# KirillHit/snn_for_object_detection

Hardware: AMD Instinct MI355X
Metric: event-frames/sec (BxT) SODa-3M GEN1 304x240 fwd+bwd (higher is better)
Workload: dtype f32 (16-bit split products)

## Files before the change

### snn_for_object_detection_amd/csrc/conv_halo.hip

```cpp
#include <stdlib.h>
#include <type_traits>
#include "conv_common.h"

namespace {

constexpr int HBM_ = 128;
constexpr int HCELLS = 288;
constexpr int HPIECE = HCELLS * 64;
constexpr int NPASS = HCELLS / 32;
static_assert(NPASS == 9, "one halo staging pass per tap");

struct HaloGeom {
    int64_t ldx, ldy, ld_add, ld_add2;
    int N, H, W, Cin, Cout;
    int PW, PH;
    int G;
    int group_cells;
    int tiles_per_group, tiles, tiles_per_xcd, ntiles_n;
    unsigned magic_pw, magic_ph;
    int out_vec;
    double* bn_partial;
    int OH, OW;
    int tiles_x, tiles_img;
    float x_th;
};

__device__ __forceinline__ unsigned udiv_small(unsigned n, unsigned magic) { return __umulhi(n, magic); }

template <bool F16>
__device__ __forceinline__ void split4(const f32x4& v, u32x2& hi, u32x2& lo) {
#pragma unroll
    for (int e = 0; e < 4; e += 2) {
        if constexpr (F16) {
            const float a = v[e] * kF16ActScale, b = v[e + 1] * kF16ActScale;
            const f16x2 ph = __builtin_convertvector(f32x2{a, b}, f16x2);
            const f16x2 pl = __builtin_convertvector(f32x2{a - (float)ph[0], b - (float)ph[1]}, f16x2);
            hi[e >> 1] = __builtin_bit_cast(unsigned, ph);
            lo[e >> 1] = __builtin_bit_cast(unsigned, pl);
        } else {
            f32x2 rest = {v[e], v[e + 1]};
            const bf16x2 ph = __builtin_convertvector(rest, bf16x2);
            const unsigned bits = __builtin_bit_cast(unsigned, ph);
            rest[0] -= __builtin_bit_cast(float, bits << 16);
            rest[1] -= __builtin_bit_cast(float, bits & 0xffff0000u);
            const bf16x2 pl = __builtin_convertvector(rest, bf16x2);
            hi[e >> 1] = bits;
            lo[e >> 1] = __builtin_bit_cast(unsigned, pl);
        }
    }
}

__device__ __forceinline__ double partner8(double v) {
    const u32x2 u = __builtin_bit_cast(u32x2, v);
    const u32x2 o = {(unsigned)__builtin_amdgcn_update_dpp(0, (int)u[0], 0x128, 0xf, 0xf, false),
                     (unsigned)__builtin_amdgcn_update_dpp(0, (int)u[1], 0x128, 0xf, 0xf, false)};
    return __builtin_bit_cast(double, o);
}
__device__ __forceinline__ double partner16(double v) {
    const u32x2 u = __builtin_bit_cast(u32x2, v);
    const u32x2 o = {__builtin_amdgcn_permlane16_swap(u[0], u[0], false, false)[0],
                     __builtin_amdgcn_permlane16_swap(u[1], u[1], false, false)[0]};
    return __builtin_bit_cast(double, o);
}
__device__ __forceinline__ double partner32(double v) {
    const u32x2 u = __builtin_bit_cast(u32x2, v);
    const u32x2 o = {__builtin_amdgcn_permlane32_swap(u[0], u[0], false, false)[0],
                     __builtin_amdgcn_permlane32_swap(u[1], u[1], false, false)[0]};
    return __builtin_bit_cast(double, o);
}

__device__ __forceinline__ int cell_slot_off(int cell, int slot) { return cell * 64 + ((slot ^ ((cell >> 2) & 3)) << 4); }


constexpr int RTH = 4, RTW = 32, RPITCH = RTW + 2, RCELLS = (RTH + 2) * RPITCH;

template <int CO, bool F16, int ABL = 0, bool RECT = false, bool SBF = false, bool XSP = false>
__global__ __launch_bounds__(kThreads, 2) void k_conv_halo3(const float* __restrict__ x,
                                                           const unsigned char* __restrict__ wimg,
                                                           float* __restrict__ y, HaloGeom g,
                                                           const float* __restrict__ addend,
                                                           const float* __restrict__ addend2) {
    constexpr int WM = CO == 32 ? 4 : 2, WN = 4 / WM, TM = CO == 32 ? 1 : 2, TN = CO == 32 ? 1 : CO / 64;
    static_assert(CO == 32 || CO == 64 || CO == 128, "channel tile");
    constexpr int BTILE = (CO / 32) * 4096;
    constexpr int NDMA = (CO / 32) * 4 / 4;
    constexpr int ES = SBF ? 2 : 4;
    static_assert(!SBF || (!F16 && ABL == 0), "bf16 storage: bf16 MFMA, plain variant");
    static_assert(!XSP || (F16 && !SBF && ABL == 0), "spikes from potentials: the forward arithmetic, plain variant");
    constexpr int HC = RECT ? (RCELLS + 31) / 32 * 32 : HCELLS;
    constexpr int HP = HC * 64;
    constexpr int RED_BYTES = (F16 || SBF) ? 4 * (CO == 128 ? 64 : 32) * 16 : 0;
    __shared__ __attribute__((aligned(16))) unsigned char smem[2 * HP + 2 * BTILE + RED_BYTES];
    unsigned char* Aimg = smem;
    unsigned char* Bimg = smem + 2 * HP;

    const int tid = threadIdx.x, lane = tid & 63;
    const int wave = __builtin_amdgcn_readfirstlane(tid >> 6);
    const int wm = wave / WN, wn = wave % WN;
    const int r = lane & 31, h = lane >> 5;

    const int bq = blockIdx.x >> 3;
    const int tile = (blockIdx.x & 7) * g.tiles_per_xcd + bq / g.ntiles_n;
    if (tile >= g.tiles) return;
    const int n0c = (bq % g.ntiles_n) * CO;
    int grp, kt, c0 = 0, x0 = 0, y0 = 0, n0, nb;
    [[maybe_unused]] int ty = 0, tx = 0;
    if constexpr (RECT) {
        n0 = tile / g.tiles_img;
        const int rem = tile - n0 * g.tiles_img;
        ty = rem / g.tiles_x;
        tx = rem - ty * g.tiles_x;
        grp = n0 / g.G;
        kt = (n0 - grp * g.G) * g.tiles_img + rem;
        nb = n0;
    } else {
        grp = tile / g.tiles_per_group;
        kt = tile - grp * g.tiles_per_group;
        c0 = kt * HBM_;
        const int R0g = c0 / g.PW;
        x0 = c0 - R0g * g.PW;
        const int ng = R0g / g.PH;
        y0 = R0g - ng * g.PH;
        n0 = grp * g.G + ng;
        nb = n0 > 0 ? n0 - 1 : 0;
    }
    const int pitch = RECT ? RPITCH : g.PW;

    const int quad = tid & 7;
    const int64_t ipix = (int64_t)g.H * g.W;
    const int64_t xbytes = ((((int64_t)g.N - nb) * ipix - 1) * g.ldx + g.Cin) * ES;
    __amdgpu_buffer_rsrc_t rs_x = __builtin_amdgcn_make_buffer_rsrc(
        reinterpret_cast<char*>(const_cast<float*>(x)) + (int64_t)nb * ipix * g.ldx * ES, 0,
        xbytes > 0x7fffffffLL ? 0x7fffffff : (int)xbytes, 0x00020000);
    unsigned voff[NPASS];
    int awr[NPASS];
#pragma unroll
    for (int p = 0; p < NPASS; ++p) {
        const int cell = p * 32 + (tid >> 3);
        int xx, yy, n;
        bool ok;
        if constexpr (RECT) {
            const int rr = cell / RPITCH, cc = cell - rr * RPITCH;
            yy = ty * RTH - 1 + rr;
            xx = tx * RTW - 1 + cc;
            n = n0;
            ok = cell < RCELLS && yy >= 0 && yy < g.H && xx >= 0 && xx < g.W;
        } else {
            const unsigned u = (unsigned)(x0 + cell + g.PW - 1);
            const unsigned dR = udiv_small(u, g.magic_pw);
            xx = (int)(u - dR * g.PW);
            const unsigned v = (unsigned)(y0 + (int)dR + g.PH - 2);
            const unsigned dn = udiv_small(v, g.magic_ph);
            yy = (int)(v - dn * g.PH);
            n = n0 - 1 + (int)dn;
            ok = n >= 0 && n < g.N && xx < g.W && yy < g.H;
        }
        const int64_t pix = (int64_t)(n - nb) * ipix + (int64_t)yy * g.W + xx;
        voff[p] = ok ? (unsigned)((pix * g.ldx + quad * 4) * ES) : 0x80000000u;
        awr[p] = cell_slot_off(cell, quad >> 1) + (quad & 1) * 8;
    }

    int cellbase[TM];
#pragma unroll
    for (int i = 0; i < TM; ++i)
        cellbase[i] = RECT ? (wm * TM + i + 1) * RPITCH + 1 + r : g.PW + 1 + (wm * TM + i) * 32 + r;
    const int nchunks = g.Cin >> 5;
    const int co_tiles = g.Cout >> 5;
    const unsigned char* wsrc = wimg + (int64_t)(n0c >> 5) * 4096 + lane * 16;
    const unsigned lds_b = (unsigned)(size_t)(__attribute__((address_space(3))) unsigned char*)Bimg;
    auto dma_b = [&](int kk, int buf) {
        if constexpr (SBF)
            if (wave & 1) return;
        const int chunk = kk / 9, tap = kk - chunk * 9;
        const unsigned char* src = wsrc + ((int64_t)(tap * nchunks + chunk) * co_tiles) * 4096 + wave * 1024;
        const unsigned dst = lds_b + buf * BTILE + wave * 1024;
#pragma unroll
        for (int q = 0; q < NDMA; ++q) {
            unsigned keep;
            asm volatile("s_mov_b32 %0, m0\n\ts_mov_b32 m0, %2\n\ts_nop 0\n\tglobal_load_lds_dwordx4 %1, off\n\ts_mov_b32 m0, %0"
                         : "=&s"(keep)
                         : "v"(src + q * 4096), "s"(__builtin_amdgcn_readfirstlane(dst + q * 4096))
                         : "memory");
        }
    };

    using PReg = typename std::conditional<SBF, u32x2, f32x4>::type;
    PReg pf[NPASS];
    auto store_halo = [&]() {
#pragma unroll
        for (int p = 0; p < NPASS; ++p) {
            if constexpr (RECT)
                if (p * 32 >= HC) continue;
            if constexpr (SBF) {
                *reinterpret_cast<u32x2*>(Aimg + awr[p]) = pf[p];
            } else if constexpr (XSP) {
                const u32x2 hi = {(pf[p][0] > g.x_th ? 0x4C00u : 0u) | (pf[p][1] > g.x_th ? 0x4C000000u : 0u),
                                  (pf[p][2] > g.x_th ? 0x4C00u : 0u) | (pf[p][3] > g.x_th ? 0x4C000000u : 0u)};
                *reinterpret_cast<u32x2*>(Aimg + awr[p]) = hi;
            } else {
                u32x2 hi, lo;
                split4<F16>(pf[p], hi, lo);
                *reinterpret_cast<u32x2*>(Aimg + awr[p]) = hi;
                *reinterpret_cast<u32x2*>(Aimg + HP + awr[p]) = lo;
            }
        }
    };
    auto load_pass = [&](int off) -> PReg {
        if constexpr (SBF) return __builtin_bit_cast(u32x2, __builtin_amdgcn_raw_buffer_load_b64(rs_x, off, 0, 0));
        else return __builtin_bit_cast(f32x4, __builtin_amdgcn_raw_buffer_load_b128(rs_x, off, 0, 0));
    };

    f32x16 acc[TM][TN];
#pragma unroll
    for (int i = 0; i < TM; ++i)
#pragma unroll
        for (int j = 0; j < TN; ++j)
#pragma unroll
            for (int e = 0; e < 16; ++e) acc[i][j][e] = 0.f;

    auto kstep = [&](int tapoff, const unsigned char* Bb) {
#pragma unroll
        for (int ks = 0; ks < 2; ++ks) {
            bf16x8 ah[TM], al[TM], bh[TN], bl[TN];
#pragma unroll
            for (int i = 0; i < TM; ++i) {
                const int off = cell_slot_off(cellbase[i] + tapoff, 2 * ks + h);
                if constexpr (ABL & 16) {
                    if (i == 0 && ks == 0) ah[0] = *reinterpret_cast<const bf16x8*>(Aimg + off);
                    ah[i] = ah[0];
                    al[i] = ah[0];
                    continue;
                }
                ah[i] = *reinterpret_cast<const bf16x8*>(Aimg + off);
                if constexpr (!SBF && !XSP) al[i] = *reinterpret_cast<const bf16x8*>(Aimg + HP + off);
            }
#pragma unroll
            for (int j = 0; j < TN; ++j) {
                const int off = (wn * TN + j) * 4096 + ks * 2048 + lane * 16;
                bh[j] = *reinterpret_cast<const bf16x8*>(Bb + off);
                if constexpr (!SBF) bl[j] = *reinterpret_cast<const bf16x8*>(Bb + off + 1024);
            }
#pragma unroll
            for (int i = 0; i < TM; ++i)
#pragma unroll
                for (int j = 0; j < TN; ++j) {
                    if constexpr (SBF) {
                        acc[i][j] = __builtin_amdgcn_mfma_f32_32x32x16_bf16(ah[i], bh[j], acc[i][j], 0, 0, 0);
                    } else if constexpr (XSP) {
                        const f16x8 xah = __builtin_bit_cast(f16x8, ah[i]);
                        const f16x8 xbh = __builtin_bit_cast(f16x8, bh[j]), xbl = __builtin_bit_cast(f16x8, bl[j]);
                        acc[i][j] = __builtin_amdgcn_mfma_f32_32x32x16_f16(xah, xbl, acc[i][j], 0, 0, 0);
                        acc[i][j] = __builtin_amdgcn_mfma_f32_32x32x16_f16(xah, xbh, acc[i][j], 0, 0, 0);
                    } else if constexpr (F16) {
                        const f16x8 xah = __builtin_bit_cast(f16x8, ah[i]), xal = __builtin_bit_cast(f16x8, al[i]);
                        const f16x8 xbh = __builtin_bit_cast(f16x8, bh[j]), xbl = __builtin_bit_cast(f16x8, bl[j]);
                        acc[i][j] = __builtin_amdgcn_mfma_f32_32x32x16_f16(xal, xbh, acc[i][j], 0, 0, 0);
                        acc[i][j] = __builtin_amdgcn_mfma_f32_32x32x16_f16(xah, xbl, acc[i][j], 0, 0, 0);
                        acc[i][j] = __builtin_amdgcn_mfma_f32_32x32x16_f16(xah, xbh, acc[i][j], 0, 0, 0);
                    } else {
                        acc[i][j] = __builtin_amdgcn_mfma_f32_32x32x16_bf16(al[i], bh[j], acc[i][j], 0, 0, 0);
                        acc[i][j] = __builtin_amdgcn_mfma_f32_32x32x16_bf16(ah[i], bl[j], acc[i][j], 0, 0, 0);
                        acc[i][j] = __builtin_amdgcn_mfma_f32_32x32x16_bf16(ah[i], bh[j], acc[i][j], 0, 0, 0);
                    }
                }
        }
    };

    dma_b(0, 0);
#pragma unroll
    for (int p = 0; p < NPASS; ++p) pf[p] = load_pass((int)voff[p]);
    store_halo();
    asm volatile("s_waitcnt vmcnt(0) lgkmcnt(0)\n\ts_barrier" ::: "memory");

    const int nk = nchunks * 9;
#pragma unroll 1
    for (int chunk = 0; chunk < nchunks; ++chunk) {
        const bool more = chunk + 1 < nchunks;
        const int cbytes = (chunk + 1) * 32 * ES;
#pragma unroll
        for (int tap = 0; tap < 9; ++tap) {
            const int kk = chunk * 9 + tap;
            const int cur = kk & 1;
            if constexpr (!(ABL & 1))
                if (kk + 1 < nk) dma_b(kk + 1, cur ^ 1);
            __builtin_amdgcn_sched_barrier(0);
            if constexpr (!(ABL & 4)) {
                if (more) pf[tap] = load_pass((int)(voff[tap] + (unsigned)cbytes));
            }
            __builtin_amdgcn_sched_barrier(0);
            const int kh = tap / 3, kw = tap - 3 * kh;
            kstep((kh - 1) * pitch + (kw - 1), Bimg + cur * BTILE);
            if constexpr (ABL & 2) asm volatile("" ::: "memory");
            else if constexpr (ABL & 4) asm volatile("s_waitcnt vmcnt(0) lgkmcnt(0)\n\ts_barrier" ::: "memory");
            else asm volatile("s_waitcnt vmcnt(0) lgkmcnt(0)\n\ts_barrier" ::: "memory");
        }
        if (more) {
            store_halo();
            asm volatile("s_waitcnt lgkmcnt(0)\n\ts_barrier" ::: "memory");
        }
    }

    constexpr int EW = TN * 32 + 4;
    constexpr int LPR = TN * 8;
    constexpr int RPP = 64 / LPR;
    float* stage = reinterpret_cast<float*>(smem) + wave * 32 * EW;
    const bool ovec = g.out_vec != 0;
    const int lrow = lane / LPR, c4 = (lane % LPR) * 4;
    const int nch = n0c + wn * TN * 32 + c4;
    const int cells_left = g.group_cells - c0;
    double ssum[4] = {0.0, 0.0, 0.0, 0.0}, qsum[4] = {0.0, 0.0, 0.0, 0.0};
    const bool stats = (F16 || SBF) && g.bn_partial != nullptr;
    auto cell_pixel = [&](int m, int64_t& pix) -> bool {
        int xx, yy, n;
        bool ok;
        if constexpr (RECT) {
            yy = ty * RTH + (m >> 5);
            xx = tx * RTW + (m & 31);
            n = n0;
            ok = yy < g.H && xx < g.W && nch < g.Cout;
        } else {
            const unsigned u = (unsigned)(x0 + m);
            const unsigned dR = udiv_small(u, g.magic_pw);
            xx = (int)(u - dR * g.PW);
            const unsigned v = (unsigned)(y0 + (int)dR);
            const unsigned dn = udiv_small(v, g.magic_ph);
            yy = (int)(v - dn * g.PH);
            n = n0 + (int)dn;
            ok = m < cells_left && xx < g.W && yy < g.H && n < g.N && nch < g.Cout;
        }
        pix = ((int64_t)n * g.H + yy) * g.W + xx;
        return ok;
    };
    typedef SnnStore<SBF> St;
    constexpr int NPS = 32 / RPP;
    const bool prefetch_add = ovec && (addend != nullptr || addend2 != nullptr) && !(ABL & 8);
#pragma unroll
    for (int i = 0; i < TM; ++i) {
        f32x4 pa1[NPS], pa2[NPS];
        int64_t ppix[NPS];
        unsigned okmask = 0;
        if (prefetch_add) {
#pragma unroll
            for (int pass = 0; pass < NPS; ++pass) {
                const bool ok = cell_pixel((wm * TM + i) * 32 + pass * RPP + lrow, ppix[pass]);
                okmask |= ok ? 1u << pass : 0u;
                const int64_t pc = ok ? ppix[pass] : 0;
                const int nc = ok ? nch : 0;
                const f32x4 zero = {0.f, 0.f, 0.f, 0.f};
                pa1[pass] = addend ? St::ld4_last(addend, pc * g.ld_add + nc) : zero;
                pa2[pass] = addend2 ? St::ld4_last(addend2, pc * g.ld_add2 + nc) : zero;
            }
        }
#pragma unroll
        for (int j = 0; j < TN; ++j)
#pragma unroll
            for (int e = 0; e < 16; ++e)
                stage[((e & 3) + 8 * (e >> 2) + 4 * h) * EW + j * 32 + r] = F16 ? acc[i][j][e] * kF16Unscale : acc[i][j][e];
        asm volatile("s_waitcnt lgkmcnt(0)" ::: "memory");
        if (prefetch_add) {
#pragma unroll
            for (int pass = 0; pass < NPS; ++pass) {
                f32x4 val = *reinterpret_cast<const f32x4*>(&stage[(pass * RPP + lrow) * EW + c4]);
                if (addend) val += pa1[pass];
                if (addend2) val += pa2[pass];
                if ((okmask >> pass) & 1u) St::st4(y, ppix[pass] * g.ldy + nch, val);
            }
            asm volatile("s_waitcnt lgkmcnt(0)" ::: "memory");
            continue;
        }
#pragma unroll
        for (int pass = 0; pass < NPS; ++pass) {
            const int row = pass * RPP + lrow;
            int64_t pix;
            const bool ok = cell_pixel((wm * TM + i) * 32 + row, pix);
            f32x4 val = *reinterpret_cast<const f32x4*>(&stage[row * EW + c4]);
            if (!ok) continue;
            if constexpr (ABL & 8) {
                asm volatile("" :: "v"(val[0]), "v"(val[1]), "v"(val[2]), "v"(val[3]));
                continue;
            }
            if (ovec) {
                if (addend) val += St::ld4_last(addend, pix * g.ld_add + nch);
                if (addend2) val += St::ld4_last(addend2, pix * g.ld_add2 + nch);
                St::st4(y, pix * g.ldy + nch, val);
            } else {
#pragma unroll
                for (int q = 0; q < 4; ++q) {
                    float o = val[q];
                    if (addend) o += St::ld1(addend, pix * g.ld_add + nch + q);
                    if (addend2) o += St::ld1(addend2, pix * g.ld_add2 + nch + q);
                    St::st1(y, pix * g.ldy + nch + q, o);
                }
            }
            if (stats) {
#pragma unroll
                for (int q = 0; q < 4; ++q) {
                    const double d = (double)val[q];
                    ssum[q] += d;
                    qsum[q] = fma(d, d, qsum[q]);
                }
            }
        }
        asm volatile("s_waitcnt lgkmcnt(0)" ::: "memory");
    }
    if (stats) {
#pragma unroll
        for (int q = 0; q < 4; ++q) {
            if constexpr (LPR <= 8) {
                ssum[q] += partner8(ssum[q]);
                qsum[q] += partner8(qsum[q]);
            }
            ssum[q] += partner16(ssum[q]);
            qsum[q] += partner16(qsum[q]);
            ssum[q] += partner32(ssum[q]);
            qsum[q] += partner32(qsum[q]);
        }
        double* red = reinterpret_cast<double*>(smem + 2 * HP + 2 * BTILE);
        if (lane >= 48 && lane < 48 + LPR) {
#pragma unroll
            for (int q = 0; q < 4; ++q) {
                red[((wave * LPR + lane - 48) * 4 + q) * 2 + 0] = ssum[q];
                red[((wave * LPR + lane - 48) * 4 + q) * 2 + 1] = qsum[q];
            }
        }
        __syncthreads();
        if (tid < CO) {
            const int wn_ = tid / (TN * 32), cc = tid % (TN * 32);
            double s = 0.0, q2 = 0.0;
#pragma unroll
            for (int wm_ = 0; wm_ < WM; ++wm_) {
                const double* src = red + (((wm_ * WN + wn_) * LPR * 4) + cc) * 2;
                s += src[0];
                q2 += src[1];
            }
            if (n0c + tid < g.Cout) {
                double* dstp = g.bn_partial + snn_bn_partial_index(grp, kt, n0c + tid, g.tiles_per_group, g.Cout);
                dstp[0] = s;
                dstp[1] = q2;
            }
        }
    }
}

constexpr int SPITCH = RTW + 1, SCELLS = (RTH + 1) * SPITCH;
template <bool SBF = false, bool RECT = false>
__global__ __launch_bounds__(kThreads, 2) void k_conv_s2dgrad3(const float* __restrict__ x,
                                                              const unsigned char* __restrict__ wimg,
                                                              float* __restrict__ y,
                                                              HaloGeom g, const float* __restrict__ addend,
                                                              const float* __restrict__ addend2) {
    constexpr int CO = 64, TN = 2;
    constexpr int ES = SBF ? 2 : 4;
    constexpr int BTILE = (CO / 32) * 4096;
    constexpr int NDMA = (CO / 32) * 4 / 4;
    __shared__ __attribute__((aligned(16))) unsigned char smem[2 * HPIECE + 2 * BTILE];
    unsigned char* Aimg = smem;
    unsigned char* Bimg = smem + 2 * HPIECE;

    const int tid = threadIdx.x, lane = tid & 63;
    const int wave = __builtin_amdgcn_readfirstlane(tid >> 6);
    const int r = lane & 31, h = lane >> 5;

    const int bq = blockIdx.x >> 3;
    const int tile = (blockIdx.x & 7) * g.tiles_per_xcd + bq / g.ntiles_n;
    if (tile >= g.tiles) return;
    const int n0c = (bq % g.ntiles_n) * CO;
    int c0 = 0, x0 = 0, y0 = 0, n0;
    [[maybe_unused]] int ty = 0, tx = 0;
    if constexpr (RECT) {
        n0 = tile / g.tiles_img;
        const int rem = tile - n0 * g.tiles_img;
        ty = rem / g.tiles_x;
        tx = rem - ty * g.tiles_x;
    } else {
        c0 = tile * HBM_;
        const int R0g = c0 / g.PW;
        x0 = c0 - R0g * g.PW;
        n0 = R0g / g.PH;
        y0 = R0g - n0 * g.PH;
    }
    const int nb = n0;
    const int pitch = RECT ? SPITCH : g.PW;

    const int quad = tid & 7;
    const int64_t ipix = (int64_t)g.H * g.W;
    const int64_t xbytes = ((((int64_t)g.N - nb) * ipix - 1) * g.ldx + g.Cin) * ES;
    __amdgpu_buffer_rsrc_t rs_x = __builtin_amdgcn_make_buffer_rsrc(
        reinterpret_cast<char*>(const_cast<float*>(x)) + (int64_t)nb * ipix * g.ldx * ES, 0,
        xbytes > 0x7fffffffLL ? 0x7fffffff : (int)xbytes, 0x00020000);
    unsigned voff[NPASS];
    int awr[NPASS];
#pragma unroll
    for (int p = 0; p < NPASS; ++p) {
        const int cell = p * 32 + (tid >> 3);
        int xx, yy, n;
        bool ok;
        if constexpr (RECT) {
            const int rr = cell / SPITCH, cc = cell - rr * SPITCH;
            yy = ty * RTH + rr;
            xx = tx * RTW + cc;
            n = n0;
            ok = cell < SCELLS && xx < g.W && yy < g.H;
        } else {
            const unsigned u = (unsigned)(x0 + cell);
            const unsigned dR = udiv_small(u, g.magic_pw);
            xx = (int)(u - dR * g.PW);
            const unsigned v = (unsigned)(y0 + (int)dR);
            const unsigned dn = udiv_small(v, g.magic_ph);
            yy = (int)(v - dn * g.PH);
            n = n0 + (int)dn;
            ok = n < g.N && xx < g.W && yy < g.H;
        }
        const int64_t pix = (int64_t)(n - nb) * ipix + (int64_t)yy * g.W + xx;
        voff[p] = ok ? (unsigned)((pix * g.ldx + quad * 4) * ES) : 0x80000000u;
        awr[p] = cell_slot_off(cell, quad >> 1) + (quad & 1) * 8;
    }
    const int cellbase = RECT ? wave * SPITCH + r : wave * 32 + r;
    const int nchunks = g.Cin >> 5;
    const int co_tiles = g.Cout >> 5;
    const unsigned char* wsrc = wimg + (int64_t)(n0c >> 5) * 4096 + lane * 16;
    const unsigned lds_b = (unsigned)(size_t)(__attribute__((address_space(3))) unsigned char*)Bimg;
    auto dma_b = [&](int kk, int buf) {
        if constexpr (SBF)
            if (wave & 1) return;
        const int chunk = kk / 9, tap = kk - chunk * 9;
        const unsigned char* src = wsrc + ((int64_t)((8 - tap) * nchunks + chunk) * co_tiles) * 4096 + wave * 1024;
        const unsigned dst = lds_b + buf * BTILE + wave * 1024;
#pragma unroll
        for (int q = 0; q < NDMA; ++q) {
            unsigned keep;
            asm volatile("s_mov_b32 %0, m0\n\ts_mov_b32 m0, %2\n\ts_nop 0\n\tglobal_load_lds_dwordx4 %1, off\n\ts_mov_b32 m0, %0"
                         : "=&s"(keep)
                         : "v"(src + q * 4096), "s"(__builtin_amdgcn_readfirstlane(dst + q * 4096))
                         : "memory");
        }
    };
    using PReg = typename std::conditional<SBF, u32x2, f32x4>::type;
    PReg pf[NPASS];
    auto store_halo = [&]() {
#pragma unroll
        for (int p = 0; p < NPASS; ++p) {
            if constexpr (SBF) {
                *reinterpret_cast<u32x2*>(Aimg + awr[p]) = pf[p];
            } else {
                u32x2 hi, lo;
                split4<false>(pf[p], hi, lo);
                *reinterpret_cast<u32x2*>(Aimg + awr[p]) = hi;
                *reinterpret_cast<u32x2*>(Aimg + HPIECE + awr[p]) = lo;
            }
        }
    };
    auto load_pass = [&](int off) -> PReg {
        if constexpr (SBF) return __builtin_bit_cast(u32x2, __builtin_amdgcn_raw_buffer_load_b64(rs_x, off, 0, 0));
        else return __builtin_bit_cast(f32x4, __builtin_amdgcn_raw_buffer_load_b128(rs_x, off, 0, 0));
    };
    f32x16 acc[4][TN];
#pragma unroll
    for (int c = 0; c < 4; ++c)
#pragma unroll
        for (int j = 0; j < TN; ++j)
#pragma unroll
            for (int e = 0; e < 16; ++e) acc[c][j][e] = 0.f;

    auto kstep = [&](int tapoff, const unsigned char* Bb, f32x16 (&a)[TN]) {
#pragma unroll
        for (int ks = 0; ks < 2; ++ks) {
            const int off = cell_slot_off(cellbase + tapoff, 2 * ks + h);
            const bf16x8 ah = *reinterpret_cast<const bf16x8*>(Aimg + off);
            bf16x8 al = ah;
            if constexpr (!SBF) al = *reinterpret_cast<const bf16x8*>(Aimg + HPIECE + off);
#pragma unroll
            for (int j = 0; j < TN; ++j) {
                const int boff = j * 4096 + ks * 2048 + lane * 16;
                const bf16x8 bh = *reinterpret_cast<const bf16x8*>(Bb + boff);
                if constexpr (!SBF) {
                    const bf16x8 bl = *reinterpret_cast<const bf16x8*>(Bb + boff + 1024);
                    a[j] = __builtin_amdgcn_mfma_f32_32x32x16_bf16(al, bh, a[j], 0, 0, 0);
                    a[j] = __builtin_amdgcn_mfma_f32_32x32x16_bf16(ah, bl, a[j], 0, 0, 0);
                }
                a[j] = __builtin_amdgcn_mfma_f32_32x32x16_bf16(ah, bh, a[j], 0, 0, 0);
            }
        }
    };

    dma_b(0, 0);
#pragma unroll
    for (int p = 0; p < NPASS; ++p) pf[p] = load_pass((int)voff[p]);
    store_halo();
    asm volatile("s_waitcnt vmcnt(0) lgkmcnt(0)\n\ts_barrier" ::: "memory");

    const int nk = nchunks * 9;
#pragma unroll 1
    for (int chunk = 0; chunk < nchunks; ++chunk) {
        const bool more = chunk + 1 < nchunks;
        const int cbytes = (chunk + 1) * 32 * ES;
#pragma unroll
        for (int tap = 0; tap < 9; ++tap) {
            const int kk = chunk * 9 + tap;
            const int cur = kk & 1;
            if (kk + 1 < nk) dma_b(kk + 1, cur ^ 1);
            __builtin_amdgcn_sched_barrier(0);
            if (more) pf[tap] = load_pass((int)(voff[tap] + (unsigned)cbytes));
            __builtin_amdgcn_sched_barrier(0);
            const int kh = tap / 3, kw = tap - 3 * kh;
            const int ph = kh == 1 ? 0 : 1, pw = kw == 1 ? 0 : 1;
            const int dh = kh == 0 ? 1 : 0, dw = kw == 0 ? 1 : 0;
            kstep(dh * pitch + dw, Bimg + cur * BTILE, acc[2 * ph + pw]);
            asm volatile("s_waitcnt vmcnt(0) lgkmcnt(0)\n\ts_barrier" ::: "memory");
        }
        if (more) {
            store_halo();
            asm volatile("s_waitcnt lgkmcnt(0)\n\ts_barrier" ::: "memory");
        }
    }

    constexpr int EW = TN * 32 + 4, LPR = TN * 8, RPP = 64 / LPR;
    float* stage = reinterpret_cast<float*>(smem) + wave * 32 * EW;
    const bool ovec = g.out_vec != 0;
    const int lrow = lane / LPR, c4 = (lane % LPR) * 4;
    const int nch = n0c + c4;
    const int cells_left = g.group_cells - c0;
#pragma unroll
    for (int cls = 0; cls < 4; ++cls) {
        const int ph = cls >> 1, pw = cls & 1;
#pragma unroll
        for (int j = 0; j < TN; ++j)
#pragma unroll
            for (int e = 0; e < 16; ++e)
                stage[((e & 3) + 8 * (e >> 2) + 4 * h) * EW + j * 32 + r] = acc[cls][j][e];
        asm volatile("s_waitcnt lgkmcnt(0)" ::: "memory");
#pragma unroll
        for (int pass = 0; pass < 32 / RPP; ++pass) {
            const int row = pass * RPP + lrow;
            const int m = wave * 32 + row;
            int aa, bb, n;
            bool inside;
            if constexpr (RECT) {
                aa = ty * RTH + wave;
                bb = tx * RTW + row;
                n = n0;
                inside = true;
            } else {
                const unsigned u = (unsigned)(x0 + m);
                const unsigned dR = udiv_small(u, g.magic_pw);
                bb = (int)(u - dR * g.PW);
                const unsigned v = (unsigned)(y0 + (int)dR);
                const unsigned dn = udiv_small(v, g.magic_ph);
                aa = (int)(v - dn * g.PH);
                n = n0 + (int)dn;
                inside = m < cells_left && n < g.N;
            }
            const int hi = 2 * aa + ph, wi = 2 * bb + pw;
            const bool ok = inside && bb < g.W && aa < g.H && hi < g.OH && wi < g.OW && nch < g.Cout;
            f32x4 val = *reinterpret_cast<const f32x4*>(&stage[row * EW + c4]);
            if (!ok) continue;
            const int64_t pix = ((int64_t)n * g.OH + hi) * g.OW + wi;
            typedef SnnStore<SBF> St;
            if (ovec) {
                if (addend) val += St::ld4_last(addend, pix * g.ld_add + nch);
                if (addend2) val += St::ld4_last(addend2, pix * g.ld_add2 + nch);
                St::st4(y, pix * g.ldy + nch, val);
            } else {
#pragma unroll
                for (int q = 0; q < 4; ++q) {
                    float o = val[q];
                    if (addend) o += St::ld1(addend, pix * g.ld_add + nch + q);
                    if (addend2) o += St::ld1(addend2, pix * g.ld_add2 + nch + q);
                    St::st1(y, pix * g.ldy + nch + q, o);
                }
            }
        }
        asm volatile("s_waitcnt lgkmcnt(0)" ::: "memory");
    }
}

template <bool F16>
__global__ void k_weight_frag_image(const float* __restrict__ flat_src, unsigned char* __restrict__ flat_dst,
                                    const int64_t* __restrict__ table, int flip) {
    const int64_t* row = table + (int64_t)blockIdx.y * 4;
    const float* src = flat_src + row[0];
    unsigned char* dst = flat_dst + row[1];
    const int O = (int)row[2], I = (int)row[3];
    const int ot_n = O >> 5, ic_n = I >> 5;
    const int64_t total = (int64_t)9 * ic_n * ot_n * 2 * 64;
    for (int64_t idx = (int64_t)blockIdx.x * blockDim.x + threadIdx.x; idx < total; idx += (int64_t)gridDim.x * blockDim.x) {
        const int lane = (int)(idx & 63);
        const int ks = (int)((idx >> 6) & 1);
        int64_t rest = idx >> 7;
        const int ot = (int)(rest % ot_n); rest /= ot_n;
        const int ic = (int)(rest % ic_n);
        const int tap = (int)(rest / ic_n);
        const int r = lane & 31, h = lane >> 5;
        const int st = flip ? 8 - tap : tap;
        const float* p = src + ((int64_t)(ot * 32 + r) * 9 + st) * I + ic * 32 + ks * 16 + h * 8;
        const f32x4 v0 = *reinterpret_cast<const f32x4*>(p), v1 = *reinterpret_cast<const f32x4*>(p + 4);
        u32x4 hi, lo;
#pragma unroll
// ... 55 lines not shown
static void plan_grid(HaloPlan& p) {
    if (p.tiles * (int64_t)p.ntiles_n + 8 >= 0x7fffffffLL) {
        p.mode = 0;
        return;
    }
    p.tiles_per_xcd = (int)snn_ceil_div(p.tiles, 8);
    const int64_t grid = (int64_t)p.tiles_per_xcd * 8 * p.ntiles_n;
    if (grid > 0x7fffffffLL) p.mode = 0;
    p.grid = (int)grid;
}
static HaloPlan halo_plan(int64_t N, int H, int W, int Cin, int Cout, int G) {
    HaloPlan p = {};
    p.mode = halo_mode(N, H, W, Cin, Cout);
    if (p.mode == 0 || G <= 0 || N % G != 0) return HaloPlan{};
    p.G = G;
    p.co_tile = Cout % 128 == 0 ? 128 : (Cout % 64 == 0 ? 64 : 32);
    p.ntiles_n = Cout / p.co_tile;
    p.tiles_x = (int)snn_ceil_div(W, RTW);
    p.tiles_img = p.tiles_x * (int)snn_ceil_div(H, RTH);
    int64_t tiles;
    if (p.mode == 2) {
        p.tiles_per_group = G * p.tiles_img;
        tiles = N * (int64_t)p.tiles_img;
    } else {
        const int64_t group_cells = (int64_t)G * (H + 1) * (W + 1);
        p.group_cells = (int)group_cells;
        p.tiles_per_group = (int)snn_ceil_div(group_cells, HBM_);
        tiles = (N / G) * p.tiles_per_group;
    }
    if (tiles >= 0x7fffffffLL) return HaloPlan{};
    p.tiles = (int)tiles;
    plan_grid(p);
    return p;
}
static HaloPlan s2dgrad_plan(int64_t N, int H, int W, int Cin, int Ho, int Wo, int Cout) {
    HaloPlan p = {};
    if (!s2dgrad_shape_ok(N, H, W, Cin, Ho, Wo, Cout)) return p;
    p.mode = s2dgrad_rect(Wo) ? 2 : 1;
    p.G = (int)N;
    p.co_tile = 64;
    p.ntiles_n = Cin / 64;
    p.tiles_x = (int)snn_ceil_div(Wo, RTW);
    p.tiles_img = p.tiles_x * (int)snn_ceil_div(Ho, RTH);
    if (p.mode == 2) {
        p.tiles_per_group = p.tiles_img;
        p.tiles = (int)(N * p.tiles_img);
    } else {
        const int64_t cells = N * (int64_t)(Ho + 1) * (Wo + 1);
        p.group_cells = (int)cells;
        p.tiles_per_group = (int)snn_ceil_div(cells, HBM_);
        p.tiles = p.tiles_per_group;
    }
    plan_grid(p);
    return p;
}
static int plan_out(const HaloPlan& p, int* out) {
    const int v[7] = {p.mode, p.co_tile, p.tiles, p.tiles_per_group, p.tiles_per_xcd, p.ntiles_n, p.grid};
    for (int i = 0; i < 7; ++i) out[i] = v[i];
    return p.mode == 0 ? 1 : 0;
}

static HaloGeom halo_geom(const HaloPlan& hp, int64_t N, int H, int W, int Cin, int64_t ld_in, int OH, int OW, int Cout,
                          const void* out, int64_t ld_out, const void* addend, int64_t ld_add, const void* addend2,
                          int64_t ld_add2, bool bf16, double* bn_partial, float x_th) {
    HaloGeom g = {};
    g.ldx = ld_in; g.ldy = ld_out; g.ld_add = ld_add; g.ld_add2 = ld_add2;
    g.N = (int)N; g.H = H; g.W = W; g.Cin = Cin; g.Cout = Cout;
    g.OH = OH; g.OW = OW;
    g.PW = W + 1; g.PH = H + 1;
    g.G = hp.G;
    g.tiles_x = hp.tiles_x;
    g.tiles_img = hp.tiles_img;
    g.group_cells = hp.group_cells;
    g.tiles_per_group = hp.tiles_per_group;
    g.tiles = hp.tiles;
    g.ntiles_n = hp.ntiles_n;
    g.tiles_per_xcd = hp.tiles_per_xcd;
    g.magic_pw = magic_u32(g.PW); g.magic_ph = magic_u32(g.PH);
    g.out_vec = multiples(4, {ld_out, addend ? ld_add : 0, addend2 ? ld_add2 : 0}) && aligned(bf16 ? 8 : 16, {out, addend, addend2});
    g.bn_partial = bn_partial;
    g.x_th = x_th;
    return g;
}
}

extern "C" int snn_conv3x3_s2_dgrad_supported(int64_t N, int H, int W, int Cin, int Ho, int Wo, int Cout) {
    return s2dgrad_shape_ok(N, H, W, Cin, Ho, Wo, Cout) ? 1 : 0;
}

extern "C" int snn_conv3x3_s2_dgrad(const float* dy, int64_t lddy, const void* wt_image, float* dx, int64_t lddx, int64_t N,
                                    int H, int W, int Cin, int Ho, int Wo, int Cout, const float* addend, int64_t ld_addend,
                                    const float* addend2, int64_t ld_addend2, int precision, void* stream) {
    SNN_REQUIRE(dy && wt_image && dx, "snn_conv3x3_s2_dgrad: null pointer");
    SNN_REQUIRE(precision == SNN_PREC_BF16X3 || precision == SNN_PREC_BF16S,
                "snn_conv3x3_s2_dgrad: precision must be SNN_PREC_BF16X3 or SNN_PREC_BF16S (got %d)", precision);
    const bool sbf = precision == SNN_PREC_BF16S;
    SNN_REQUIRE(s2dgrad_shape_ok(N, H, W, Cin, Ho, Wo, Cout),
                "snn_conv3x3_s2_dgrad: shape not covered (N %lld, %dx%d -> %dx%d, %d -> %d channels; ask "
                "snn_conv3x3_s2_dgrad_supported)", (long long)N, H, W, Ho, Wo, Cin, Cout);
    SNN_REQUIRE(lddy >= Cout && lddx >= Cin && lddy % 4 == 0, "snn_conv3x3_s2_dgrad: bad pixel strides (%lld, %lld)",
                (long long)lddy, (long long)lddx);
    SNN_REQUIRE(aligned(sbf ? 8 : 16, {dy}) && aligned(16, {wt_image}),
                "snn_conv3x3_s2_dgrad: dy (16 bytes; 8 for bf16) and the weight image (16) must be aligned");
    SNN_REQUIRE(!addend || ld_addend >= Cin, "snn_conv3x3_s2_dgrad: addend pixel stride smaller than channel count");
    SNN_REQUIRE(!addend2 || ld_addend2 >= Cin, "snn_conv3x3_s2_dgrad: addend2 pixel stride smaller than channel count");
    const HaloPlan hp = s2dgrad_plan(N, H, W, Cin, Ho, Wo, Cout);
    SNN_REQUIRE(hp.mode != 0, "snn_conv3x3_s2_dgrad: grid too large");
    const bool rect = hp.mode == 2;
    if (rect)
        SNN_REQUIRE((int64_t)Ho * Wo * lddy * 4 < 0x7fffffffLL, "snn_conv3x3_s2_dgrad: a dy image must span less than 2 GiB");
    else
        SNN_REQUIRE((int64_t)4 * Ho * Wo * lddy * 4 < 0x7fffffffLL, "snn_conv3x3_s2_dgrad: four dy images must span less than 2 GiB");
    const HaloGeom g = halo_geom(hp, N, Ho, Wo, Cout, lddy, H, W, Cin, dx, lddx, addend, ld_addend, addend2, ld_addend2, sbf,
                                 nullptr, 0.0f);
    dispatch(
        [&](auto SBF, auto RECT) {
            hipLaunchKernelGGL((k_conv_s2dgrad3<SBF(), RECT()>), dim3((unsigned)hp.grid), dim3(kThreads), 0, (hipStream_t)stream,
                               dy, static_cast<const unsigned char*>(wt_image), dx, g, addend, addend2);
            return true;
        },
        Flag{sbf}, Flag{rect});
    SNN_CHECK_LAUNCH("snn_conv3x3_s2_dgrad");
    return 0;
}

extern "C" int snn_conv3x3_s2_dgrad_plan(int64_t N, int H, int W, int Cin, int Ho, int Wo, int Cout, int* out) {
    if (!out) return 1;
    return plan_out(s2dgrad_plan(N, H, W, Cin, Ho, Wo, Cout), out);
}

extern "C" int snn_conv3x3_halo_supported(int64_t N, int H, int W, int Cin, int Cout) {
    return halo_shape_ok(N, H, W, Cin, Cout) ? 1 : 0;
}

extern "C" int snn_conv3x3_halo_plan(int64_t N, int H, int W, int Cin, int Cout, int frames_per_step, int* out) {
    if (!out) return 1;
    return plan_out(halo_plan(N, H, W, Cin, Cout, frames_per_step > 0 ? frames_per_step : (int)N), out);
}

extern "C" int64_t snn_conv3x3_halo_bn_chunks(int frames_per_step, int H, int W) {
    if (W + 1 <= 79) return snn_ceil_div((int64_t)frames_per_step * (H + 1) * (W + 1), HBM_);
    return (int64_t)frames_per_step * snn_ceil_div(H, RTH) * snn_ceil_div(W, RTW);
}

extern "C" size_t snn_weight_frag_image_bytes(int O, int I) { return (size_t)9 * O * I * 4; }

extern "C" int snn_weight_frag_image_batched(const float* flat_src, void* flat_dst, const int64_t* table, int n,
                                             int max_groups, int flip, int precision, void* stream) {
    SNN_REQUIRE(flat_src && flat_dst && table && n > 0 && max_groups > 0, "snn_weight_frag_image_batched: bad arguments");
    SNN_REQUIRE(precision == SNN_PREC_FP16X3 || precision == SNN_PREC_BF16X3,
                "snn_weight_frag_image: precision must be SNN_PREC_FP16X3 (forward) or SNN_PREC_BF16X3 (data gradient)");
    SNN_REQUIRE(aligned(16, {flat_src, flat_dst}), "snn_weight_frag_image: buffers must be 16-byte aligned");
    int64_t bx = snn_ceil_div(max_groups, kThreads);
    if (bx > 64) bx = 64;
    dim3 grid((unsigned)bx, (unsigned)n);
    dispatch(
        [&](auto F16) {
            hipLaunchKernelGGL(k_weight_frag_image<F16()>, grid, dim3(kThreads), 0, (hipStream_t)stream, flat_src,
                               static_cast<unsigned char*>(flat_dst), table, flip);
            return true;
        },
        Flag{precision == SNN_PREC_FP16X3});
    SNN_CHECK_LAUNCH("snn_weight_frag_image_batched");
    return 0;
}

static int conv3x3_halo_impl(const float* x, int64_t ldx, const void* w_image, float* y, int64_t ldy, int64_t N, int H,
                             int W, int Cin, int Cout, const float* addend, int64_t ld_addend, const float* addend2,
                             int64_t ld_addend2, double* bn_partial, int frames_per_step, int* bn_layout,
                             int precision, void* stream, bool xsp, float x_th) {
    SNN_REQUIRE(x && w_image && y, "snn_conv3x3_halo: null pointer");
    SNN_REQUIRE(precision == SNN_PREC_FP16X3 || precision == SNN_PREC_BF16X3 || precision == SNN_PREC_BF16S,
                "snn_conv3x3_halo: precision must be SNN_PREC_FP16X3, SNN_PREC_BF16X3 or SNN_PREC_BF16S (got %d)", precision);
    const bool sbf = precision == SNN_PREC_BF16S;
    SNN_REQUIRE(halo_shape_ok(N, H, W, Cin, Cout),
                "snn_conv3x3_halo: shape not covered (N %lld, %dx%d, %d -> %d channels; ask snn_conv3x3_halo_supported)",
                (long long)N, H, W, Cin, Cout);
    SNN_REQUIRE(ldx >= Cin && ldy >= Cout && ldx % 4 == 0, "snn_conv3x3_halo: bad pixel strides (%lld, %lld)",
                (long long)ldx, (long long)ldy);
    SNN_REQUIRE(aligned(sbf ? 8 : 16, {x}) && aligned(16, {w_image}),
                "snn_conv3x3_halo: x (16 bytes; 8 for bf16) and the weight image (16) must be aligned");
    SNN_REQUIRE(!addend || ld_addend >= Cout, "snn_conv3x3_halo: addend pixel stride smaller than channel count");
    SNN_REQUIRE(!addend2 || ld_addend2 >= Cout, "snn_conv3x3_halo: addend2 pixel stride smaller than channel count");
    SNN_REQUIRE(!bn_partial || ((precision == SNN_PREC_FP16X3 || sbf) && bn_layout && frames_per_step > 0 &&
                                N % frames_per_step == 0 && !addend && !addend2),
                "snn_conv3x3_halo: statistics need the forward arithmetic, bn_layout, no addend and a frames_per_step "
                "that divides N (%lld frames, %d per step)", (long long)N, frames_per_step);
    SNN_REQUIRE((int64_t)4 * H * W * ldx * 4 < 0x7fffffffLL, "snn_conv3x3_halo: four images must span less than 2 GiB");
    if (bn_layout) bn_layout[0] = bn_layout[1] = 0;
    const HaloPlan hp = halo_plan(N, H, W, Cin, Cout, bn_partial ? frames_per_step : (int)N);
    SNN_REQUIRE(hp.mode != 0, "snn_conv3x3_halo: grid too large");
    const bool rect = hp.mode == 2;
    if (rect) SNN_REQUIRE((int64_t)H * W * ldx * 4 < 0x7fffffffLL, "snn_conv3x3_halo: an image must span less than 2 GiB");
    const HaloGeom g = halo_geom(hp, N, H, W, Cin, ldx, H, W, Cout, y, ldy, addend, ld_addend, addend2, ld_addend2, sbf,
                                 bn_partial, x_th);
    if (bn_partial) bn_layout[0] = g.tiles_per_group;
    const dim3 grid((unsigned)hp.grid);
    const unsigned char* wi = static_cast<const unsigned char*>(w_image);
#ifdef SNN_TUNING
    if (const char* e = snn_tuning_env("SNN_HALO_ABL")) {
        const bool launched = dispatch(
            [&](auto ABL, auto CO) {
                hipLaunchKernelGGL((k_conv_halo3<CO(), true, ABL()>), grid, dim3(kThreads), 0, (hipStream_t)stream, x, wi, y, g,
                                   addend, addend2);
                return true;
            },
            OneOf<1, 2, 4, 8, 16, 3, 7, 15, 31>{atoi(e)}, OneOf<64, 128>{hp.co_tile == 128 ? 128 : 64});
        if (launched) {
            SNN_CHECK_LAUNCH("snn_conv3x3_halo");
            return 0;
        }
    }
#endif
    enum { kPieces = 0, kBf16Storage = 1, kSpikes = 2 };
    const bool f16 = precision == SNN_PREC_FP16X3;
    dispatch(
        [&](auto CO, auto RECT, auto OPERAND, auto F16) {
            if constexpr (OPERAND() == kPieces || F16() == (OPERAND() == kSpikes)) {
                hipLaunchKernelGGL((k_conv_halo3<CO(), F16(), 0, RECT(), OPERAND() == kBf16Storage, OPERAND() == kSpikes>), grid,
                                   dim3(kThreads), 0, (hipStream_t)stream, x, wi, y, g, addend, addend2);
            }
            return true;
        },
        OneOf<32, 64, 128>{hp.co_tile}, Flag{rect}, OneOf<0, 1, 2>{xsp ? kSpikes : (sbf ? kBf16Storage : kPieces)}, Flag{f16});
    SNN_CHECK_LAUNCH(xsp ? "snn_conv3x3_halo_spikes" : "snn_conv3x3_halo");
    return 0;
}

extern "C" int snn_conv3x3_halo(const float* x, int64_t ldx, const void* w_image, float* y, int64_t ldy, int64_t N, int H,
                                int W, int Cin, int Cout, const float* addend, int64_t ld_addend, const float* addend2,
                                int64_t ld_addend2, double* bn_partial, int frames_per_step, int* bn_layout,
                                int precision, void* stream) {
    return conv3x3_halo_impl(x, ldx, w_image, y, ldy, N, H, W, Cin, Cout, addend, ld_addend, addend2, ld_addend2, bn_partial,
                             frames_per_step, bn_layout, precision, stream, false, 0.0f);
}

extern "C" int snn_conv3x3_halo_spikes(const float* vdec, int64_t ld, float v_th, const void* w_image, float* y, int64_t ldy,
                                       int64_t N, int H, int W, int Cin, int Cout, double* bn_partial, int frames_per_step,
                                       int* bn_layout, void* stream) {
    SNN_REQUIRE(v_th >= 0.0f, "snn_conv3x3_halo_spikes: a negative threshold would turn padding into spikes");
    return conv3x3_halo_impl(vdec, ld, w_image, y, ldy, N, H, W, Cin, Cout, nullptr, 0, nullptr, 0, bn_partial,
                             frames_per_step, bn_layout, SNN_PREC_FP16X3, stream, true, v_th);
}
```

Measured before the change: 7387.

## Use a three-slot weight DMA ring in halo conv and stride-2 dgrad kernels

Adds an NBUF template parameter so the 3x3 halo conv and stride-2 dgrad kernels can keep weight tiles in a ring of three LDS slots, prefetching two taps ahead. The per-tap wait then only drains down to the newest DMA batch (vmcnt(NDMA)) instead of waiting for all outstanding loads. This hides weight-load latency behind the MFMA steps. The cost is an extra LDS tile, with the statistics reduction region moved into a reused slot, which may reduce occupancy. The chunk loop is also split so the last chunk is a compile-time variant, and an env var can force depth two.

```diff
diff --git a/snn_for_object_detection_amd/csrc/conv_halo.hip b/snn_for_object_detection_amd/csrc/conv_halo.hip
--- a/snn_for_object_detection_amd/csrc/conv_halo.hip
+++ b/snn_for_object_detection_amd/csrc/conv_halo.hip
@@ -74,7 +74,7 @@
 
 constexpr int RTH = 4, RTW = 32, RPITCH = RTW + 2, RCELLS = (RTH + 2) * RPITCH;
 
-template <int CO, bool F16, int ABL = 0, bool RECT = false, bool SBF = false, bool XSP = false>
+template <int CO, bool F16, int ABL = 0, bool RECT = false, bool SBF = false, bool XSP = false, int NBUF = 2>
 __global__ __launch_bounds__(kThreads, 2) void k_conv_halo3(const float* __restrict__ x,
                                                            const unsigned char* __restrict__ wimg,
                                                            float* __restrict__ y, HaloGeom g,
@@ -89,8 +89,12 @@
     static_assert(!XSP || (F16 && !SBF && ABL == 0), "spikes from potentials: the forward arithmetic, plain variant");
     constexpr int HC = RECT ? (RCELLS + 31) / 32 * 32 : HCELLS;
     constexpr int HP = HC * 64;
+    static_assert(NBUF == 2 || (NBUF == 3 && CO <= 64 && !SBF && ABL == 0),
+                  "ring of three: every wave issues the same DMA count (not bf16 storage), and a third 16 KiB tile does not fit twice");
     constexpr int RED_BYTES = (F16 || SBF) ? 4 * (CO == 128 ? 64 : 32) * 16 : 0;
-    __shared__ __attribute__((aligned(16))) unsigned char smem[2 * HP + 2 * BTILE + RED_BYTES];
+    static_assert(RED_BYTES <= BTILE, "statistics region inside one ring slot");
+    constexpr int RED_OFF = NBUF == 3 ? 2 * HP : 2 * HP + 2 * BTILE;
+    __shared__ __attribute__((aligned(16))) unsigned char smem[2 * HP + NBUF * BTILE + (NBUF == 3 ? 0 : RED_BYTES)];
     unsigned char* Aimg = smem;
     unsigned char* Bimg = smem + 2 * HP;
 
@@ -168,10 +172,9 @@
     const int co_tiles = g.Cout >> 5;
     const unsigned char* wsrc = wimg + (int64_t)(n0c >> 5) * 4096 + lane * 16;
     const unsigned lds_b = (unsigned)(size_t)(__attribute__((address_space(3))) unsigned char*)Bimg;
-    auto dma_b = [&](int kk, int buf) {
+    auto dma_ct = [&](int chunk, int tap, int buf) {
         if constexpr (SBF)
             if (wave & 1) return;
-        const int chunk = kk / 9, tap = kk - chunk * 9;
         const unsigned char* src = wsrc + ((int64_t)(tap * nchunks + chunk) * co_tiles) * 4096 + wave * 1024;
         const unsigned dst = lds_b + buf * BTILE + wave * 1024;
 #pragma unroll
@@ -182,6 +185,10 @@
                          : "v"(src + q * 4096), "s"(__builtin_amdgcn_readfirstlane(dst + q * 4096))
                          : "memory");
         }
+    };
+    auto dma_b = [&](int kk, int buf) {
+        const int chunk = kk / 9;
+        dma_ct(chunk, kk - chunk * 9, buf);
     };
 
     using PReg = typename std::conditional<SBF, u32x2, f32x4>::type;
@@ -270,35 +277,55 @@
 #pragma unroll
     for (int p = 0; p < NPASS; ++p) pf[p] = load_pass((int)voff[p]);
     store_halo();
-    asm volatile("s_waitcnt vmcnt(0) lgkmcnt(0)\n\ts_barrier" ::: "memory");
+    if constexpr (NBUF == 3) {
+        __builtin_amdgcn_sched_barrier(0);
+        dma_ct(0, 1, 1);
+        asm volatile("s_waitcnt vmcnt(%0) lgkmcnt(0)\n\ts_barrier" ::"n"(NDMA) : "memory");
+    } else {
+        asm volatile("s_waitcnt vmcnt(0) lgkmcnt(0)\n\ts_barrier" ::: "memory");
+    }
 
     const int nk = nchunks * 9;
+    auto chunk_pass = [&](int chunk, auto MORE) {
+        constexpr bool more = decltype(MORE)::value;
+        [[maybe_unused]] const int cbytes = (chunk + 1) * 32 * ES;
+#pragma unroll
+        for (int tap = 0; tap < 9; ++tap) {
+            const int kh = tap / 3, kw = tap - 3 * kh;
+            if constexpr (NBUF == 3) {
+                if constexpr (more) pf[tap] = load_pass((int)(voff[tap] + (unsigned)cbytes));
+                __builtin_amdgcn_sched_barrier(0);
+                const bool ahead = tap < 7 || (tap == 7 && more);
+                if (ahead) dma_ct(tap < 7 ? chunk : chunk + 1, (tap + 2) % 9, (tap + 2) % 3);
+                __builtin_amdgcn_sched_barrier(0);
+                kstep((kh - 1) * pitch + (kw - 1), Bimg + (tap % 3) * BTILE);
+                if (ahead) asm volatile("s_waitcnt vmcnt(%0) lgkmcnt(0)\n\ts_barrier" ::"n"(NDMA) : "memory");
+                else asm volatile("s_waitcnt vmcnt(0) lgkmcnt(0)\n\ts_barrier" ::: "memory");
+            } else {
+                const int kk = chunk * 9 + tap;
+                const int cur = kk & 1;
+                if constexpr (!(ABL & 1))
+                    if (kk + 1 < nk) dma_b(kk + 1, cur ^ 1);
+                __builtin_amdgcn_sched_barrier(0);
+                if constexpr (!(ABL & 4) && more) pf[tap] = load_pass((int)(voff[tap] + (unsigned)cbytes));
+                __builtin_amdgcn_sched_barrier(0);
+                kstep((kh - 1) * pitch + (kw - 1), Bimg + cur * BTILE);
+                if constexpr (ABL & 2) asm volatile("" ::: "memory");
+                else asm volatile("s_waitcnt vmcnt(0) lgkmcnt(0)\n\ts_barrier" ::: "memory");
+            }
+        }
+        if constexpr (more) {
+            store_halo();
+            if constexpr (NBUF == 3) {
+                __builtin_amdgcn_sched_barrier(0);
+                dma_ct(chunk + 1, 1, 1);
+            }
+            asm volatile("s_waitcnt lgkmcnt(0)\n\ts_barrier" ::: "memory");
+        }
+    };
 #pragma unroll 1
-    for (int chunk = 0; chunk < nchunks; ++chunk) {
-        const bool more = chunk + 1 < nchunks;
-        const int cbytes = (chunk + 1) * 32 * ES;
-#pragma unroll
-        for (int tap = 0; tap < 9; ++tap) {
-            const int kk = chunk * 9 + tap;
-            const int cur = kk & 1;
-            if constexpr (!(ABL & 1))
-                if (kk + 1 < nk) dma_b(kk + 1, cur ^ 1);
-            __builtin_amdgcn_sched_barrier(0);
-            if constexpr (!(ABL & 4)) {
-                if (more) pf[tap] = load_pass((int)(voff[tap] + (unsigned)cbytes));
-            }
-            __builtin_amdgcn_sched_barrier(0);
-            const int kh = tap / 3, kw = tap - 3 * kh;
-            kstep((kh - 1) * pitch + (kw - 1), Bimg + cur * BTILE);
-            if constexpr (ABL & 2) asm volatile("" ::: "memory");
-            else if constexpr (ABL & 4) asm volatile("s_waitcnt vmcnt(0) lgkmcnt(0)\n\ts_barrier" ::: "memory");
-            else asm volatile("s_waitcnt vmcnt(0) lgkmcnt(0)\n\ts_barrier" ::: "memory");
-        }
-        if (more) {
-            store_halo();
-            asm volatile("s_waitcnt lgkmcnt(0)\n\ts_barrier" ::: "memory");
-        }
-    }
+    for (int chunk = 0; chunk + 1 < nchunks; ++chunk) chunk_pass(chunk, std::true_type{});
+    chunk_pass(nchunks - 1, std::false_type{});
 
     constexpr int EW = TN * 32 + 4;
     constexpr int LPR = TN * 8;
@@ -415,7 +442,8 @@
             ssum[q] += partner32(ssum[q]);
             qsum[q] += partner32(qsum[q]);
         }
-        double* red = reinterpret_cast<double*>(smem + 2 * HP + 2 * BTILE);
+        static_assert(4 * 32 * EW * 4 <= RED_OFF, "accumulator staging rows end below the statistics region");
+        double* red = reinterpret_cast<double*>(smem + RED_OFF);
         if (lane >= 48 && lane < 48 + LPR) {
 #pragma unroll
             for (int q = 0; q < 4; ++q) {
@@ -443,7 +471,7 @@
 }
 
 constexpr int SPITCH = RTW + 1, SCELLS = (RTH + 1) * SPITCH;
-template <bool SBF = false, bool RECT = false>
+template <bool SBF = false, bool RECT = false, int NBUF = 2>
 __global__ __launch_bounds__(kThreads, 2) void k_conv_s2dgrad3(const float* __restrict__ x,
                                                               const unsigned char* __restrict__ wimg,
                                                               float* __restrict__ y,
@@ -453,7 +481,8 @@
     constexpr int ES = SBF ? 2 : 4;
     constexpr int BTILE = (CO / 32) * 4096;
     constexpr int NDMA = (CO / 32) * 4 / 4;
-    __shared__ __attribute__((aligned(16))) unsigned char smem[2 * HPIECE + 2 * BTILE];
+    static_assert(NBUF == 2 || (NBUF == 3 && !SBF), "ring of three: every wave issues the same DMA count");
+    __shared__ __attribute__((aligned(16))) unsigned char smem[2 * HPIECE + NBUF * BTILE];
     unsigned char* Aimg = smem;
     unsigned char* Bimg = smem + 2 * HPIECE;
 
@@ -520,10 +549,9 @@
     const int co_tiles = g.Cout >> 5;
     const unsigned char* wsrc = wimg + (int64_t)(n0c >> 5) * 4096 + lane * 16;
     const unsigned lds_b = (unsigned)(size_t)(__attribute__((address_space(3))) unsigned char*)Bimg;
-    auto dma_b = [&](int kk, int buf) {
+    auto dma_ct = [&](int chunk, int tap, int buf) {
         if constexpr (SBF)
             if (wave & 1) return;
-        const int chunk = kk / 9, tap = kk - chunk * 9;
         const unsigned char* src = wsrc + ((int64_t)((8 - tap) * nchunks + chunk) * co_tiles) * 4096 + wave * 1024;
         const unsigned dst = lds_b + buf * BTILE + wave * 1024;
 #pragma unroll
@@ -534,6 +562,10 @@
                          : "v"(src + q * 4096), "s"(__builtin_amdgcn_readfirstlane(dst + q * 4096))
                          : "memory");
         }
+    };
+    auto dma_b = [&](int kk, int buf) {
+        const int chunk = kk / 9;
+        dma_ct(chunk, kk - chunk * 9, buf);
     };
     using PReg = typename std::conditional<SBF, u32x2, f32x4>::type;
     PReg pf[NPASS];
@@ -587,32 +619,55 @@
 #pragma unroll
     for (int p = 0; p < NPASS; ++p) pf[p] = load_pass((int)voff[p]);
     store_halo();
-    asm volatile("s_waitcnt vmcnt(0) lgkmcnt(0)\n\ts_barrier" ::: "memory");
+    if constexpr (NBUF == 3) {
+        __builtin_amdgcn_sched_barrier(0);
+        dma_ct(0, 1, 1);
+        asm volatile("s_waitcnt vmcnt(%0) lgkmcnt(0)\n\ts_barrier" ::"n"(NDMA) : "memory");
+    } else {
+        asm volatile("s_waitcnt vmcnt(0) lgkmcnt(0)\n\ts_barrier" ::: "memory");
+    }
 
     const int nk = nchunks * 9;
-#pragma unroll 1
-    for (int chunk = 0; chunk < nchunks; ++chunk) {
-        const bool more = chunk + 1 < nchunks;
-        const int cbytes = (chunk + 1) * 32 * ES;
+    auto chunk_pass = [&](int chunk, auto MORE) {
+        constexpr bool more = decltype(MORE)::value;
+        [[maybe_unused]] const int cbytes = (chunk + 1) * 32 * ES;
 #pragma unroll
         for (int tap = 0; tap < 9; ++tap) {
-            const int kk = chunk * 9 + tap;
-            const int cur = kk & 1;
-            if (kk + 1 < nk) dma_b(kk + 1, cur ^ 1);
-            __builtin_amdgcn_sched_barrier(0);
-            if (more) pf[tap] = load_pass((int)(voff[tap] + (unsigned)cbytes));
-            __builtin_amdgcn_sched_barrier(0);
             const int kh = tap / 3, kw = tap - 3 * kh;
             const int ph = kh == 1 ? 0 : 1, pw = kw == 1 ? 0 : 1;
             const int dh = kh == 0 ? 1 : 0, dw = kw == 0 ? 1 : 0;
-            kstep(dh * pitch + dw, Bimg + cur * BTILE, acc[2 * ph + pw]);
-            asm volatile("s_waitcnt vmcnt(0) lgkmcnt(0)\n\ts_barrier" ::: "memory");
-        }
-        if (more) {
+            if constexpr (NBUF == 3) {
+                if constexpr (more) pf[tap] = load_pass((int)(voff[tap] + (unsigned)cbytes));
+                __builtin_amdgcn_sched_barrier(0);
+                const bool ahead = tap < 7 || (tap == 7 && more);
+                if (ahead) dma_ct(tap < 7 ? chunk : chunk + 1, (tap + 2) % 9, (tap + 2) % 3);
+                __builtin_amdgcn_sched_barrier(0);
+                kstep(dh * pitch + dw, Bimg + (tap % 3) * BTILE, acc[2 * ph + pw]);
+                if (ahead) asm volatile("s_waitcnt vmcnt(%0) lgkmcnt(0)\n\ts_barrier" ::"n"(NDMA) : "memory");
+                else asm volatile("s_waitcnt vmcnt(0) lgkmcnt(0)\n\ts_barrier" ::: "memory");
+            } else {
+                const int kk = chunk * 9 + tap;
+                const int cur = kk & 1;
+                if (kk + 1 < nk) dma_b(kk + 1, cur ^ 1);
+                __builtin_amdgcn_sched_barrier(0);
+                if constexpr (more) pf[tap] = load_pass((int)(voff[tap] + (unsigned)cbytes));
+                __builtin_amdgcn_sched_barrier(0);
+                kstep(dh * pitch + dw, Bimg + cur * BTILE, acc[2 * ph + pw]);
+                asm volatile("s_waitcnt vmcnt(0) lgkmcnt(0)\n\ts_barrier" ::: "memory");
+            }
+        }
+        if constexpr (more) {
             store_halo();
+            if constexpr (NBUF == 3) {
+                __builtin_amdgcn_sched_barrier(0);
+                dma_ct(chunk + 1, 1, 1);
+            }
             asm volatile("s_waitcnt lgkmcnt(0)\n\ts_barrier" ::: "memory");
         }
-    }
+    };
+#pragma unroll 1
+    for (int chunk = 0; chunk + 1 < nchunks; ++chunk) chunk_pass(chunk, std::true_type{});
+    chunk_pass(nchunks - 1, std::false_type{});
 
     constexpr int EW = TN * 32 + 4, LPR = TN * 8, RPP = 64 / LPR;
     float* stage = reinterpret_cast<float*>(smem) + wave * 32 * EW;
@@ -834,6 +889,19 @@
     g.x_th = x_th;
     return g;
 }
+
+static bool halo_ring_depth2_forced() {
+    static const bool depth2 = [] {
+        const char* e = getenv("SNN_HALO_DMA_DEPTH");
+        return e != nullptr && atoi(e) == 2;
+    }();
+    return depth2;
+}
+constexpr bool halo_ring3_instance(int co_tile, bool f16, bool sbf) { return !sbf && (co_tile == 32 || (co_tile == 64 && f16)); }
+static int halo_ring_depth(int co_tile, bool f16, bool sbf) {
+    return !halo_ring_depth2_forced() && halo_ring3_instance(co_tile, f16, sbf) ? 3 : 2;
+}
+static int s2dgrad_ring_depth(bool sbf) { return !halo_ring_depth2_forced() && !sbf ? 3 : 2; }
 }
 
 extern "C" int snn_conv3x3_s2_dgrad_supported(int64_t N, int H, int W, int Cin, int Ho, int Wo, int Cout) {
@@ -866,12 +934,14 @@
     const HaloGeom g = halo_geom(hp, N, Ho, Wo, Cout, lddy, H, W, Cin, dx, lddx, addend, ld_addend, addend2, ld_addend2, sbf,
                                  nullptr, 0.0f);
     dispatch(
-        [&](auto SBF, auto RECT) {
-            hipLaunchKernelGGL((k_conv_s2dgrad3<SBF(), RECT()>), dim3((unsigned)hp.grid), dim3(kThreads), 0, (hipStream_t)stream,
-                               dy, static_cast<const unsigned char*>(wt_image), dx, g, addend, addend2);
+        [&](auto SBF, auto RECT, auto NBUF) {
+            if constexpr (!(SBF() && NBUF() == 3)) {
+                hipLaunchKernelGGL((k_conv_s2dgrad3<SBF(), RECT(), NBUF()>), dim3((unsigned)hp.grid), dim3(kThreads), 0,
+                                   (hipStream_t)stream, dy, static_cast<const unsigned char*>(wt_image), dx, g, addend, addend2);
+            }
             return true;
         },
-        Flag{sbf}, Flag{rect});
+        Flag{sbf}, Flag{rect}, OneOf<2, 3>{s2dgrad_ring_depth(sbf)});
     SNN_CHECK_LAUNCH("snn_conv3x3_s2_dgrad");
     return 0;
 }
@@ -967,14 +1037,17 @@
     enum { kPieces = 0, kBf16Storage = 1, kSpikes = 2 };
     const bool f16 = precision == SNN_PREC_FP16X3;
     dispatch(
-        [&](auto CO, auto RECT, auto OPERAND, auto F16) {
-            if constexpr (OPERAND() == kPieces || F16() == (OPERAND() == kSpikes)) {
-                hipLaunchKernelGGL((k_conv_halo3<CO(), F16(), 0, RECT(), OPERAND() == kBf16Storage, OPERAND() == kSpikes>), grid,
-                                   dim3(kThreads), 0, (hipStream_t)stream, x, wi, y, g, addend, addend2);
+        [&](auto CO, auto RECT, auto OPERAND, auto F16, auto NBUF) {
+            if constexpr ((OPERAND() == kPieces || F16() == (OPERAND() == kSpikes)) &&
+                          (NBUF() == 2 || halo_ring3_instance(CO(), F16(), OPERAND() == kBf16Storage))) {
+                hipLaunchKernelGGL(
+                    (k_conv_halo3<CO(), F16(), 0, RECT(), OPERAND() == kBf16Storage, OPERAND() == kSpikes, NBUF()>), grid,
+                    dim3(kThreads), 0, (hipStream_t)stream, x, wi, y, g, addend, addend2);
             }
             return true;
         },
-        OneOf<32, 64, 128>{hp.co_tile}, Flag{rect}, OneOf<0, 1, 2>{xsp ? kSpikes : (sbf ? kBf16Storage : kPieces)}, Flag{f16});
+        OneOf<32, 64, 128>{hp.co_tile}, Flag{rect}, OneOf<0, 1, 2>{xsp ? kSpikes : (sbf ? kBf16Storage : kPieces)}, Flag{f16},
+        OneOf<2, 3>{halo_ring_depth(hp.co_tile, f16, sbf)});
     SNN_CHECK_LAUNCH(xsp ? "snn_conv3x3_halo_spikes" : "snn_conv3x3_halo");
     return 0;
 }
```

After: 7456, median of 6. No clear change (+0.9%).
